# ClashLuke/LocAtE

Measured on AMD Instinct MI355X. Metric: images/sec (G+D step) 64x64 bs=64, higher is better.
Workload: dtype f32 (contractions fp32-faithful on the matrix cores: 2 x scaled fp16 operand pieces / 3 MFMAs per slice where the operand's largest magnitude comes with it, else 3 x bf16 pieces / 6 MFMAs; fp32 accumulate); 1 GPU; LocAtE G+D step, 64x64 RGB, batch 64 per GPU (the fp32 variant - the reference's own precision - of BASELINE.json configs[1]: 64x64 RGB bs 64), self/feature attention at 16x16 and 64x64, random-init weights; global_batch=64, image_size=64, parallelism=dp1, launch=hipGraph replay, G-step generator pass on a second stream

## Files before the change

### include/locate_hip.h

```cpp
#ifndef LOCATE_HIP_H
#define LOCATE_HIP_H
#include <stddef.h>
#include <stdint.h>
#ifdef __cplusplus
extern "C" {
#endif

const char* locate_last_error(void);
int locate_abi_version(void);
int locate_device_info(char* arch_name, int name_len, int* cu_count, int* wave_size);

int locate_roottanh_fwd(const float* x, float* y, int64_t n, void* absmax , void* stream);
int locate_absmax_words(void);
int locate_roottanh_bwd(const float* x, const float* gy, float* gx, int64_t n, int accumulate, void* absmax, void* stream);
int locate_absmax(const float* x, int64_t n, void* absmax, void* stream);
int locate_act_cat_rows_fwd(const float* latent, const float* pre, float* out, int rows, int z, int w, void* stream);
int locate_act_rows_bwd(const float* pre, const float* g, int64_t g_row_stride, const float* g_add, float* gpre, int rows, int w,
                        void* stream);
int locate_add3(const float* a, int64_t a_bs, const float* b, int64_t b_bs, const float* c, int64_t c_bs, float* out, int batch,
                int64_t per, void* stream);
int locate_tanh_fwd(const float* x, float* y, int64_t n, void* stream);
int locate_tanh_bwd(const float* y, const float* gy, float* gx, int64_t n, void* stream);

size_t locate_norm_stats_workspace_bytes(void);
// ... 71 lines not shown
int locate_conv_dgrad(const int* geom, const float* gy, int64_t gy_bs, const float* panel, const float* scale,
                      int scale_group_batch, int scale_stride, const float* bias, float* gx, int64_t gx_bs, void* workspace,
                      void* counters, int precision, const void* gy_absmax, const void* act_epilogue, void* stream);
size_t locate_conv_wgrad_workspace_bytes(const int* geom);
int locate_conv_wgrad_partials(const int* geom);
int locate_conv_wgrad(const int* geom, const float* x, int64_t x_bs, const float* gy, int64_t gy_bs, float* gw,
                      const float* w_ref, const float* inv_scale, int scale_group_batch, int scale_stride,
                      double* inner_partial, void* workspace, int precision, const void* x_absmax, const void* gy_absmax,
                      void* deferred_reduce, void* stream);
int locate_conv_wgrad_group_partials(const int* geom, int groups);
size_t locate_conv_wgrad_group_workspace_bytes(const int* geom, int groups);
size_t locate_slab_reduce_record_bytes(void);
int locate_slab_reduce_max(void);
int locate_slab_reduce_record_blocks(const void* record);
int locate_slab_reduce_batch(const void* records, int n, void* stream);

size_t locate_wgrad_batch_record_bytes(void);
int locate_wgrad_batch_max(void);
int locate_wgrad_batch_record(const int* geom, const float* x, int64_t x_bs, const float* gy, int64_t gy_bs, float* gw,
                              const float* w_ref, const float* inv_scale, int scale_group_batch, int scale_stride,
                              double* inner_partial, void* record);
int locate_wgrad_batch(const void* records, int n, void* stream);

int locate_dwconv_fwd(const int* geom, const float* x, int64_t x_bs, const float* w, const float* scale, int scale_group_batch,
                      int scale_stride, float* y, int64_t y_bs, void* stream);
int locate_dwconv_dgrad(const int* geom, const float* gy, int64_t gy_bs, const float* w, const float* scale,
                        int scale_group_batch, int scale_stride, float* gx, int64_t gx_bs, void* stream);
size_t locate_dwconv_wgrad_workspace_bytes(const int* geom);
int locate_dwconv_wgrad_partials(const int* geom);
int locate_dwconv_wgrad(const int* geom, const float* big, int64_t big_bs, const float* small, int64_t small_bs, float* gw,
// ... 48 lines not shown
```

### locate_amd/_lib.py

```python
import ctypes
import os

import torch

_HERE = os.path.dirname(os.path.abspath(__file__))
LIB_PATH = os.path.join(_HERE, "csrc", "liblocate_hip_dbg.so" if os.environ.get("LOCATE_HIP_DEBUG_LIBRARY") == "1"
                        else "liblocate_hip.so")

c_p = ctypes.c_void_p
c_i = ctypes.c_int
c_i64 = ctypes.c_int64
c_f = ctypes.c_float
c_d = ctypes.c_double
c_sz = ctypes.c_size_t
c_ip = ctypes.POINTER(ctypes.c_int)

PROTOTYPES = {
    "locate_last_error": (ctypes.c_char_p, []),
    "locate_abi_version": (c_i, []),
    "locate_device_info": (c_i, [ctypes.c_char_p, c_i, c_ip, c_ip]),
    "locate_roottanh_fwd": (c_i, [c_p, c_p, c_i64, c_p, c_p]),
    "locate_roottanh_bwd": (c_i, [c_p, c_p, c_p, c_i64, c_i, c_p, c_p]),
    "locate_act_cat_rows_fwd": (c_i, [c_p, c_p, c_p, c_i, c_i, c_i, c_p]),
    "locate_act_rows_bwd": (c_i, [c_p, c_p, c_i64, c_p, c_p, c_i, c_i, c_p]),
# ... 48 lines not shown
    "locate_conv_pack_panels": (c_i, [c_p, c_i, c_i, c_i, c_i, c_p]),
    "locate_conv_pack_job_is_direct": (c_i, [c_p]),
    "locate_conv_pack_job_is_window": (c_i, [c_p]),
    "locate_conv_win_ok": (c_i, [c_ip, c_i, c_i64, c_p]),
    "locate_conv_win_workspace_bytes": (c_sz, [c_ip, c_i]),
    "locate_conv_fwd_workspace_bytes": (c_sz, [c_ip]),
    "locate_conv_counter_bytes": (c_sz, []),
    "locate_conv_fwd": (c_i, [c_ip, c_p, c_i64, c_p, c_p, c_i, c_i, c_p, c_p, c_i64, c_p, c_p, c_i, c_p, c_p, c_p]),
    "locate_conv_dgrad_workspace_bytes": (c_sz, [c_ip]),
    "locate_conv_dgrad": (c_i, [c_ip, c_p, c_i64, c_p, c_p, c_i, c_i, c_p, c_p, c_i64, c_p, c_p, c_i, c_p, c_p, c_p]),
    "locate_conv_wgrad_workspace_bytes": (c_sz, [c_ip]),
    "locate_conv_wgrad_partials": (c_i, [c_ip]),
    "locate_conv_wgrad": (c_i, [c_ip, c_p, c_i64, c_p, c_i64, c_p, c_p, c_p, c_i, c_i, c_p, c_p, c_i, c_p, c_p, c_p, c_p]),
    "locate_conv_wgrad_group_partials": (c_i, [c_ip, c_i]),
    "locate_conv_wgrad_group_workspace_bytes": (c_sz, [c_ip, c_i]),
    "locate_slab_reduce_record_bytes": (c_sz, []),
    "locate_slab_reduce_max": (c_i, []),
    "locate_slab_reduce_record_blocks": (c_i, [c_p]),
    "locate_slab_reduce_batch": (c_i, [c_p, c_i, c_p]),
    "locate_dwconv_fwd": (c_i, [c_ip, c_p, c_i64, c_p, c_p, c_i, c_i, c_p, c_i64, c_p]),
    "locate_dwconv_dgrad": (c_i, [c_ip, c_p, c_i64, c_p, c_p, c_i, c_i, c_p, c_i64, c_p]),
    "locate_dwconv_wgrad_workspace_bytes": (c_sz, [c_ip]),
    "locate_dwconv_wgrad_partials": (c_i, [c_ip]),
    "locate_dwconv_wgrad": (c_i, [c_ip, c_p, c_i64, c_p, c_i64, c_p, c_p, c_p, c_i, c_i, c_p, c_p, c_p]),
    "locate_groupdot_fwd": (c_i, [c_p, c_i64, c_p, c_p, c_i, c_i, c_p, c_i, c_i, c_i, c_p]),
    "locate_groupdot_dgrad": (c_i, [c_p, c_p, c_p, c_i, c_i, c_p, c_i64, c_i, c_i, c_i, c_p]),
    "locate_groupdot_wgrad_partials": (c_i, [c_i, c_i]),
    "locate_groupdot_wgrad": (c_i, [c_p, c_i64, c_p, c_p, c_p, c_p, c_i, c_i, c_p, c_i, c_i, c_i, c_p]),
    "locate_fin_record_bytes": (c_sz, []),
    "locate_fin_sn_dot_partials": (c_i, [c_i, c_i, c_i]),
# ... 13 lines not shown
    "locate_g_loss": (c_i, [c_p, c_i, c_p, c_p, c_p]),
    "locate_input_param_record_bytes": (c_sz, []),
    "locate_input_mean_blocks": (c_i, [c_i, c_i]),
    "locate_input_workspace_bytes": (c_sz, [c_i, c_i, c_i]),
    "locate_input_transform": (c_i, [c_p, c_i, c_i, c_i, c_p, c_p, c_i, c_i, c_p, c_i, c_i, c_i, c_p, c_i, c_p, c_p, c_p, c_p]),
    "locate_image_range_workspace_bytes": (c_sz, []),
    "locate_image_range": (c_i, [c_p, c_i64, c_p, c_p, c_p]),
    "locate_image_grid": (c_i, [c_p, c_i, c_i, c_i, c_i, c_f, c_p, c_f, c_p, c_p, c_p]),
}


class LocateError(RuntimeError):
    pass


EXPECTED_ABI = 10


_lib = None


def lib():
    global _lib
    if _lib is None:
        if not os.path.exists(LIB_PATH):
            raise LocateError("%s is missing: run `python -m locate_amd.build` (hipcc, gfx950). "
                              "There is no CPU fallback for the MI355X kernels." % LIB_PATH)
        handle = ctypes.CDLL(LIB_PATH)
        for name, (res, args) in PROTOTYPES.items():
            fn = getattr(handle, name)
            fn.restype = res
# ... 26 lines not shown
```

### locate_amd/csrc/convwgrad.hip

```cpp
#include "igemm.h"

#define WG_BK 32

struct WgParams {
    const float* x;
    const float* gy;
    float* slab;
    long long x_bs, gy_bs;
    unsigned x_bytes;
    int B, C, H, W, M, OH, OW, KH, KW, stride, pad_h, pad_w;
    int R;
    int N;
    int chunk;
    int zper, Ng;
    unsigned q_mul, ow_mul;
    int q_s1, q_s2, ow_s1, ow_s2;
    int gscale_bg, gscale_stride;
    float* direct_out;
    const float* w_ref;
    const float* inv_scale;
    double* partial;
    const unsigned* x_absmax;
    const unsigned* g_absmax;
};


template <int WGM, int WGN, int TM, int TN>
__device__ __forceinline__ void wgrad_epilogue(const WgParams& p, f32x16 (&acc)[TM][TN], int r0, int m0, int wm, int wn, int lane,
                                               int wid, int tid) {
    const int lrow = lane >> 5, lcol = lane & 31;
    __shared__ double red[4];
    const bool direct = p.direct_out != nullptr;
    float* dst = direct ? p.direct_out : p.slab + (long long)blockIdx.z * p.M * p.R;
    const float sc = (direct && p.inv_scale && p.gscale_bg == 0) ? p.inv_scale[0] : 1.0f;
    double dot = 0.0;
    const bool want_dot = direct && p.w_ref != nullptr;
#pragma unroll
    for (int j = 0; j < TN; ++j) {
        const int r = r0 + (wn * TN + j) * 32 + lcol;
        const bool r_ok = r < p.R;
#pragma unroll
        for (int i = 0; i < TM; ++i) {
            float wref[16];
#pragma unroll
            for (int e = 0; e < 16; ++e) {
                const int m = m0 + (wm * TM + i) * 32 + (e & 3) + 8 * (e >> 2) + 4 * lrow;
                const bool ok = want_dot && r_ok && m < p.M;
                const float* wp_ = ok ? p.w_ref + (long long)m * p.R + r : p.gy;
// ... 2 lines not shown
            float part = 0.0f;
#pragma unroll
            for (int e = 0; e < 16; ++e) {
                const int m = m0 + (wm * TM + i) * 32 + (e & 3) + 8 * (e >> 2) + 4 * lrow;
                const float v = acc[i][j][e];
                part = fmaf(v, wref[e], part);
                if (r_ok && m < p.M) dst[(long long)m * p.R + r] = v * sc;
            }
            dot += (double)part;
        }
    }
    if (direct && p.partial) {
        dot = wave_sum_d(dot);
        if (lane == 0) red[wid] = dot;
        __syncthreads();
        if (tid == 0) p.partial[blockIdx.y * gridDim.x + blockIdx.x] = (red[0] + red[1]) + (red[2] + red[3]);
    }
}

template <int WGM, int WGN, int TM, int TN>
__global__ void __launch_bounds__(256) conv_wgrad_kernel(const WgParams p) {
    constexpr int BM = WGM * TM * 32;
    constexpr int BR = WGN * TN * 32;
    constexpr int G_PT = WG_BK * BM / 256;
    constexpr int X_PT = WG_BK * BR / 256;
    static_assert(WGM * WGN == 4, "four waves");

    __shared__ float Gs[2][WG_BK][BM + 1];
    __shared__ float Xs[2][WG_BK][BR + 1];
    __shared__ int rt_off[BR];
    __shared__ signed char rt_dy[BR], rt_dx[BR];

    const int tid = threadIdx.x, lane = tid & 63, wid = tid >> 6;
    const int wm = wid / WGN, wn = wid % WGN;
    const int r0 = blockIdx.x * BR, m0 = blockIdx.y * BM;
    const int taps = p.KH * p.KW;
    for (int i = tid; i < BR; i += 256) {
        const int r = r0 + i;
        if (r < p.R) {
            const int c = r / taps, t = r - c * taps;
            const int kh = t / p.KW, kw = t - kh * p.KW;
            rt_dy[i] = (signed char)(kh - p.pad_h);
            rt_dx[i] = (signed char)(kw - p.pad_w);
            rt_off[i] = c * p.H * p.W + (kh - p.pad_h) * p.W + (kw - p.pad_w);
        } else {
            rt_dy[i] = rt_dx[i] = 0;
// ... 90 lines not shown
        for (int k2 = 0; k2 < WG_BK / 2; ++k2) {
            float a[TM], b[TN];
#pragma unroll
            for (int i = 0; i < TM; ++i) a[i] = Gs[buf][k2 * 2 + lrow][(wm * TM + i) * 32 + lcol];
#pragma unroll
            for (int j = 0; j < TN; ++j) b[j] = Xs[buf][k2 * 2 + lrow][(wn * TN + j) * 32 + lcol];
#pragma unroll
            for (int i = 0; i < TM; ++i)
#pragma unroll
                for (int j = 0; j < TN; ++j) acc[i][j] = __builtin_amdgcn_mfma_f32_32x32x2f32(a[i], b[j], acc[i][j], 0, 0, 0);
        }
        if (s + 1 < nsteps) store_tiles(buf ^ 1);
        __syncthreads();
    }

    wgrad_epilogue<WGM, WGN, TM, TN>(p, acc, r0, m0, wm, wn, lane, wid, tid);
}

#define WB_BK 16
#define WB_PITCH 8

template <int WGM, int WGN, int TM, int TN, int NP>
__global__ void __launch_bounds__(256, (WGM * TM > 4 ? 2 : 3)) conv_wgrad_bx6_kernel(const WgParams p) {
    constexpr int BM = WGM * TM * 32;
    constexpr int BR = WGN * TN * 32;
    constexpr int G_PT = BM / 32;
    constexpr int X_PT = BR / 32;
    static_assert(WGM * WGN == 4, "four waves");

    constexpr int NPL = NP == 4 ? 1 : NP;
    __shared__ unsigned Gs[2][NPL][NP == 4 ? 1 : BM][WB_PITCH];
    __shared__ unsigned Xs[2][NPL][NP == 4 ? 1 : BR][WB_PITCH];
    __shared__ __attribute__((aligned(16))) unsigned short G8[2][NP == 4 ? BM : 1][8];
    __shared__ __attribute__((aligned(16))) unsigned short X8[2][NP == 4 ? BR : 1][8];

    const int tid = threadIdx.x, lane = tid & 63, wid = tid >> 6;
    const int wm = wid / WGN, wn = wid % WGN;
    const int r0 = blockIdx.x * BR, m0 = blockIdx.y * BM;
    const int taps = p.KH * p.KW;
    const int np = tid & 7, sub = tid >> 3;
    const int Q = p.OH * p.OW;

    int xoff[X_PT], xdy[X_PT], xdx[X_PT];
#pragma unroll
    for (int i = 0; i < X_PT; ++i) {
        const int r = r0 + sub + 32 * i;
        if (r < p.R) {
            const int c = r / taps, t = r - c * taps;
            const int kh = t / p.KW, kw = t - kh * p.KW;
            xdy[i] = kh - p.pad_h;
            xdx[i] = kw - p.pad_w;
            xoff[i] = 4 * (c * p.H * p.W + xdy[i] * p.W + xdx[i]);
        } else {
            xdy[i] = -(1 << 20);
            xdx[i] = 0;
            xoff[i] = 0;
        }
    }
    const __amdgpu_buffer_rsrc_t xrsrc = __builtin_amdgcn_make_buffer_rsrc(const_cast<float*>(p.x), 0, (int)p.x_bytes, 0x00020000);

    f32x16 acc[TM][TN];
#pragma unroll
    for (int i = 0; i < TM; ++i)
#pragma unroll
        for (int j = 0; j < TN; ++j)
#pragma unroll
            for (int r = 0; r < 16; ++r) acc[i][j][r] = 0.0f;

    const int zgrp = (int)blockIdx.z / p.zper;
    const int n_begin = zgrp * p.Ng + ((int)blockIdx.z - zgrp * p.zper) * p.chunk;
    int n_end = n_begin + p.chunk;
    if (n_end > (zgrp + 1) * p.Ng) n_end = (zgrp + 1) * p.Ng;

    float gs0 = 1.0f, gs1 = 1.0f, gs2 = 1.0f, gs3 = 1.0f, gsc = 1.0f;
    if (p.gscale_bg > 0) {
        const int ng = p.B / p.gscale_bg;
        gs0 = p.inv_scale[0];
        gs1 = ng > 1 ? p.inv_scale[p.gscale_stride] : 1.0f;
        gs2 = ng > 2 ? p.inv_scale[2 * p.gscale_stride] : 1.0f;
        gs3 = ng > 3 ? p.inv_scale[3 * p.gscale_stride] : 1.0f;
    }

    float g_scale = 1.0f, x_scale = 1.0f, g_unscale = 1.0f, x_unscale = 1.0f;
    if constexpr (NP == 2) {
        const float gmax = __uint_as_float(absmax_read(p.g_absmax)) * fmaxf(fmaxf(gs0, gs1), fmaxf(gs2, gs3));
// ... 149 lines not shown
        __builtin_amdgcn_sched_barrier(0);
        store_tiles(buf ^ 1);
        load_tiles(n_begin + (s + 2) * WB_BK);
        __builtin_amdgcn_sched_barrier(0);
        mfmas(HALF, NMF);
        __syncthreads();
    }
    if constexpr (NP == 2 || NP == 4) {
#pragma unroll
        for (int i = 0; i < TM; ++i)
#pragma unroll
            for (int j = 0; j < TN; ++j)
#pragma unroll
                for (int r = 0; r < 16; ++r) acc[i][j][r] = (acc[i][j][r] * g_unscale) * x_unscale;
    }
    wgrad_epilogue<WGM, WGN, TM, TN>(p, acc, r0, m0, wm, wn, lane, wid, tid);
}

template <int V>
__device__ __forceinline__ void slab_load(const float* p, float (&v)[V]) {
    if constexpr (V == 4) { const float4 t = *reinterpret_cast<const float4*>(p); v[0] = t.x; v[1] = t.y; v[2] = t.z; v[3] = t.w; }
    else v[0] = *p;
}

template <int ZP, int V>
__device__ __forceinline__ void slab_reduce_groups(const float* __restrict__ slab, float* __restrict__ out, int64_t n, int nsplit,
                                                   const float* __restrict__ w_ref, double* __restrict__ partial, int bid, int nblocks,
                                                   int groups, int zper, float* zbuf, double* gscratch) {
    float (*gzsum)[ZP][256 / ZP][V] = reinterpret_cast<float (*)[ZP][256 / ZP][V]>(zbuf);
    constexpr int TPB = 256 / ZP, EPB = TPB * V;
    const int ex = threadIdx.x % TPB, ez = threadIdx.x / TPB;
// ... 712 lines not shown
    return !path_disabled("skinny") && !skinny_wgrad_ok(g) && g.OH == 1 && g.OW == 1 && (long long)g.C * g.H * g.W < (1 << 24);
}
static dim3 onepix_wgrad_grid(const ConvGeom& g) { return dim3((g.C * g.H * g.W + 63) / 64, (g.M + skw_mt(g.M) - 1) / skw_mt(g.M)); }

enum WgradKind { WG_MAP1X1, WG_ONEPIX, WG_POINTWISE, WG_TILED };
struct WgradRoute {
    WgradKind kind;
    dim3 grid;
    int bm;
    PwPlan pw;
    int nsplit, chunk, zper;
    int64_t n;
    int partials;
    size_t ws_bytes;
    bool dots;
};

static WgradRoute wgrad_route(const ConvGeom& g, int groups) {
    WgradRoute r;
    const bool stacked = groups >= 2 && groups <= 4 && g.B % groups == 0;
    if (!stacked) groups = 0;
    r.bm = 0; r.nsplit = 1; r.chunk = 0; r.zper = 1; r.partials = 0; r.ws_bytes = 0; r.dots = false;
    r.n = (int64_t)g.M * g.C * g.KH * g.KW;
    const bool map1x1 = skinny_wgrad_ok(g);
    if (map1x1 || onepix_wgrad_ok(g)) {
        r.kind = map1x1 ? WG_MAP1X1 : WG_ONEPIX;
        r.grid = map1x1 ? skinny_wgrad_grid(g) : onepix_wgrad_grid(g);
        r.partials = (int)(r.grid.x * r.grid.y);
        return r;
    }
    r.pw = pw_plan(g, groups);
    if (r.pw.ok) {
        r.kind = WG_POINTWISE;
        if (stacked && r.pw.zper == 0) return r;
        r.nsplit = r.pw.nslab; r.chunk = r.pw.chunk; r.zper = r.pw.zper;
        r.grid = dim3(r.pw.nslab, r.pw.tiles_m * r.pw.tiles_c);
        r.dots = stacked;
    } else {
        r.kind = WG_TILED;
        int tiles;
        wgrad_plan(g, groups, &r.bm, &r.nsplit, &r.chunk, &r.zper, &tiles);
        r.grid = dim3((g.C * g.KH * g.KW + 127) / 128, (g.M + r.bm - 1) / r.bm, r.nsplit);
        r.dots = stacked && (long long)g.B * g.OH * g.OW < (1ll << 31);
        if (r.nsplit == 1) { r.partials = tiles; return r; }
    }
    r.partials = wgrad_reduce_grid(r.n, r.nsplit);
    r.ws_bytes = (size_t)r.nsplit * r.n * sizeof(float);
    return r;
}

LOCATE_API size_t locate_conv_wgrad_workspace_bytes(const int* geom) { return wgrad_route(make_geom(geom), 0).ws_bytes; }

LOCATE_API int locate_conv_wgrad_partials(const int* geom) { return wgrad_route(make_geom(geom), 0).partials; }

LOCATE_API size_t locate_wgrad_batch_record_bytes(void) { return sizeof(SkwRec); }
LOCATE_API int locate_wgrad_batch_max(void) { return SKW_MAX; }
LOCATE_API int locate_wgrad_batch_record(const int* geom, const float* x, int64_t x_bs, const float* gy, int64_t gy_bs, float* gw,
                                         const float* w_ref, const float* inv_scale, int scale_group_batch, int scale_stride,
// ... 39 lines not shown
    const WgradRoute r = wgrad_route(g, groups);
    return r.dots ? r.partials : 0;
}
LOCATE_API size_t locate_conv_wgrad_group_workspace_bytes(const int* geom, int groups) {
    const ConvGeom g = make_geom(geom);
    if (geom_check(g, "locate_conv_wgrad_group_workspace_bytes")) return 0;
    const WgradRoute r = wgrad_route(g, groups);
    return r.dots ? r.ws_bytes : 0;
}

template <int NP>
static void launch_wgrad_bx6(const WgParams& p, dim3 grid, int bm, hipStream_t st) {
    with_tile<true>(bm, [&](auto t) { using T = decltype(t); conv_wgrad_bx6_kernel<T::wgm, T::wgn, T::tm, T::tn, NP><<<grid, 256, 0, st>>>(p); });
}

LOCATE_API int locate_conv_wgrad(const int* geom, const float* x, int64_t x_bs, const float* gy, int64_t gy_bs, float* gw,
                                 const float* w_ref, const float* inv_scale, int scale_group_batch, int scale_stride,
                                 double* inner_partial, void* workspace, int precision, const void* x_absmax, const void* gy_absmax,
                                 void* deferred_reduce, void* stream) {
    const ConvGeom g = make_geom(geom);
    if (int e = geom_check(g, "locate_conv_wgrad")) return e;
    LOCATE_REQUIRE(precision >= 0 && precision <= 3, "locate_conv_wgrad: precision must be 0 (fp32-faithful, bf16 pieces), 1 (bf16 operands), 2 (fp32-faithful, fp16 pieces) or 3 (fp8 operands)");
    LOCATE_REQUIRE(precision < 2 || (x_absmax && gy_absmax), "locate_conv_wgrad: precisions 2 and 3 need the absmax words of x and gy");
    LOCATE_REQUIRE(x && gy && gw, "locate_conv_wgrad: null pointer");
    LOCATE_REQUIRE(!inner_partial || w_ref, "locate_conv_wgrad: inner_partial needs w_ref");
    const int gd = (scale_group_batch > 0 && w_ref && inner_partial && g.B % scale_group_batch == 0) ? g.B / scale_group_batch : 0;
    const WgradRoute r = wgrad_route(g, gd);
    LOCATE_REQUIRE(scale_group_batch >= 0 && (scale_group_batch == 0 || (inv_scale && g.B % scale_group_batch == 0 &&
                   g.B / scale_group_batch <= 4 && ((!w_ref && !inner_partial) || r.dots))),
                   "locate_conv_wgrad: bad group scaling arguments (per-call partials: see locate_conv_wgrad_group_partials)");
    hipStream_t st = as_stream(stream);
    if (deferred_reduce) memset(deferred_reduce, 0, sizeof(SlabRec));
    auto reduce = [&](const float* slab, const float* scale, const char* who) -> int {
        const int64_t n = r.n;
        const int nsplit = r.nsplit, zper = r.zper, rg = r.partials;
        const int zp = wgrad_reduce_zp(nsplit, n);
        if (deferred_reduce) {
            SlabRec rec;
            rec.slab = slab; rec.out = gw; rec.w_ref = w_ref; rec.inv_scale = scale; rec.partial = inner_partial;
            rec.n = n; rec.nsplit = nsplit; rec.zp = zp; rec.grid = rg; rec.block0 = 0; rec.groups = gd; rec.zper = zper;
            memcpy(deferred_reduce, &rec, sizeof(rec));
            return LOCATE_OK;
        }
        if (zp == 16) slab_reduce_kernel<16><<<rg, 256, 0, st>>>(slab, gw, n, nsplit, w_ref, scale, inner_partial, gd, zper);
        else if (zp == 4) slab_reduce_kernel<4><<<rg, 256, 0, st>>>(slab, gw, n, nsplit, w_ref, scale, inner_partial, gd, zper);
        else slab_reduce_kernel<1><<<rg, 256, 0, st>>>(slab, gw, n, nsplit, w_ref, scale, inner_partial, gd, zper);
        LOCATE_LAUNCH_CHECK(who);
        return LOCATE_OK;
    };
    if (r.kind == WG_MAP1X1) {
        skinny_wgrad_kernel<<<r.grid, 256, 0, st>>>(x, x_bs, gy, gy_bs, gw, w_ref, inv_scale, scale_group_batch, scale_stride,
                                                   inner_partial, g.B, g.M, g.C, OnePix{0, 0, 0, 0, 0, 0, 0});
        LOCATE_LAUNCH_CHECK("locate_conv_wgrad(1x1 map)");
        return LOCATE_OK;
    }
    if (r.kind == WG_ONEPIX) {
        const OnePix op = {g.H * g.W, g.W, g.KH, g.KW, g.pad_h, g.pad_w, g.C};
        skinny_wgrad_kernel<<<r.grid, 256, 0, st>>>(x, x_bs, gy, gy_bs, gw, w_ref, inv_scale, scale_group_batch, scale_stride,
// ... 24 lines not shown
            else pw_wgrad_kernel<2, 2, 2><<<grid, 256, 0, st>>>(q);
        } else if (precision == 1) {
            if (key == 0) pw_wgrad_kernel<1, 1, 1><<<grid, 256, 0, st>>>(q);
            else if (key == 1) pw_wgrad_kernel<1, 2, 1><<<grid, 256, 0, st>>>(q);
            else if (key == 2) pw_wgrad_kernel<2, 1, 1><<<grid, 256, 0, st>>>(q);
            else pw_wgrad_kernel<2, 2, 1><<<grid, 256, 0, st>>>(q);
        } else {
            if (key == 0) pw_wgrad_kernel<1, 1, 3><<<grid, 256, 0, st>>>(q);
            else if (key == 1) pw_wgrad_kernel<1, 2, 3><<<grid, 256, 0, st>>>(q);
            else if (key == 2) pw_wgrad_kernel<2, 1, 3><<<grid, 256, 0, st>>>(q);
            else pw_wgrad_kernel<2, 2, 3><<<grid, 256, 0, st>>>(q);
        }
        LOCATE_LAUNCH_CHECK("locate_conv_wgrad(pointwise)");
        return reduce(q.slab, grouped ? nullptr : inv_scale, "locate_conv_wgrad(pointwise reduce)");
    }
    const int bm = r.bm, nsplit = r.nsplit, chunk = r.chunk, zper = r.zper;
    LOCATE_REQUIRE(nsplit == 1 || workspace, "locate_conv_wgrad: split reduction needs a workspace");
    WgParams p;
    p.x = x; p.gy = gy; p.slab = static_cast<float*>(workspace); p.x_bs = x_bs; p.gy_bs = gy_bs;
    p.B = g.B; p.C = g.C; p.H = g.H; p.W = g.W; p.M = g.M; p.OH = g.OH; p.OW = g.OW; p.KH = g.KH; p.KW = g.KW;
    p.stride = g.stride; p.pad_h = g.pad_h; p.pad_w = g.pad_w;
    p.R = g.C * g.KH * g.KW; p.N = g.B * g.OH * g.OW; p.chunk = chunk;
    p.zper = zper; p.Ng = gd > 1 ? p.N / gd : p.N;
    fastdiv_make((unsigned)(g.OH * g.OW), &p.q_mul, &p.q_s1, &p.q_s2);
    fastdiv_make((unsigned)g.OW, &p.ow_mul, &p.ow_s1, &p.ow_s2);
    const bool direct = nsplit == 1;
    const bool grouped = scale_group_batch > 0;
    p.gscale_bg = scale_group_batch; p.gscale_stride = scale_stride;
    p.x_absmax = static_cast<const unsigned*>(x_absmax);
    p.g_absmax = static_cast<const unsigned*>(gy_absmax);
    p.direct_out = direct ? gw : nullptr;
    p.w_ref = direct ? w_ref : nullptr;
    p.inv_scale = (direct || grouped) ? inv_scale : nullptr;
    p.partial = direct ? inner_partial : nullptr;
    const long long x_extent = 4ll * ((long long)(g.B - 1) * x_bs + (long long)g.C * g.H * g.W);
    p.x_bytes = (unsigned)x_extent;
    const bool pairs_ok = ((g.OH * g.OW) & 1) == 0 && (g.OW & 1) == 0 && (gy_bs & 1) == 0 && (chunk & 1) == 0 &&
                          (reinterpret_cast<uintptr_t>(gy) & 7) == 0 && x_extent > 0 && x_extent < (1ll << 31) - (1 << 20);
    LOCATE_REQUIRE(bm != 192 || pairs_ok, "locate_conv_wgrad: layers with M %% 192 == 0 on even maps take the paired-load kernels - gy must be 8-byte aligned with an even batch stride");
    const bool bx6 = pairs_ok && (precision == 1 || precision == 3 || !path_disabled("wbx6"));
    if (bx6 && precision == 3) launch_wgrad_bx6<4>(p, grid, bm, st);
    else if (bx6 && precision == 1) launch_wgrad_bx6<1>(p, grid, bm, st);
    else if (bx6 && precision == 2) launch_wgrad_bx6<2>(p, grid, bm, st);
    else if (bx6) launch_wgrad_bx6<3>(p, grid, bm, st);
    else
        with_tile<false>(bm, [&](auto t) { using T = decltype(t); conv_wgrad_kernel<T::wgm, T::wgn, T::tm, T::tn><<<grid, 256, 0, st>>>(p); });
    LOCATE_LAUNCH_CHECK("locate_conv_wgrad(gemm)");
    if (!direct) return reduce(p.slab, grouped ? nullptr : inv_scale, "locate_conv_wgrad(reduce)");
    return LOCATE_OK;
}

LOCATE_API size_t locate_slab_reduce_record_bytes(void) { return sizeof(SlabRec); }
LOCATE_API int locate_slab_reduce_max(void) { return SLAB_MAX; }
LOCATE_API int locate_slab_reduce_record_blocks(const void* record) {
    if (!record) return 0;
    SlabRec r;
    memcpy(&r, record, sizeof(r));
    return r.grid;
}
LOCATE_API int locate_slab_reduce_batch(const void* records, int n, void* stream) {
    LOCATE_REQUIRE(records && n > 0 && n <= SLAB_MAX, "locate_slab_reduce_batch: 1 .. locate_slab_reduce_max() records");
    SlabBatch b;
    memcpy(b.r, records, (size_t)n * sizeof(SlabRec));
    long long blocks = 0;
    for (int i = 0; i < n; ++i) {
        const SlabRec& r = b.r[i];
// ... 10 lines not shown
```

### locate_amd/csrc/runtime.hip

```cpp
#include "common.h"
#include <stdarg.h>
#include <stdio.h>

static thread_local char g_last_error[512] = "";

void locate_set_error(const char* fmt, ...) {
    va_list ap;
    va_start(ap, fmt);
    vsnprintf(g_last_error, sizeof(g_last_error), fmt, ap);
    va_end(ap);
}

LOCATE_API const char* locate_last_error(void) { return g_last_error; }

LOCATE_API int locate_abi_version(void) { return 10; }

LOCATE_API int locate_device_info(char* arch_name, int name_len, int* cu_count, int* wave_size) {
    int dev = 0;
    hipDeviceProp_t prop;
    if (hipGetDevice(&dev) != hipSuccess || hipGetDeviceProperties(&prop, dev) != hipSuccess) {
        locate_set_error("locate_device_info: no HIP device");
        return LOCATE_ERR_LAUNCH;
    }
    if (arch_name && name_len > 0) snprintf(arch_name, name_len, "%s", prop.gcnArchName);
    if (cu_count) *cu_count = prop.multiProcessorCount;
    if (wave_size) *wave_size = prop.warpSize;
    return LOCATE_OK;
}
```

### locate_amd/ops.py

```python
import ctypes
import os

import torch

from ._lib import check, lib

_IntArr12 = ctypes.c_int * 12


class _ActEpilogue(ctypes.Structure):
    _fields_ = [("act_out", ctypes.c_void_p), ("act_bs", ctypes.c_int64), ("lat", ctypes.c_void_p), ("lat_bs", ctypes.c_int64),
                ("lat_z", ctypes.c_int32), ("pad", ctypes.c_int32), ("mul_pre", ctypes.c_void_p), ("mul_bs", ctypes.c_int64),
                ("out_absmax", ctypes.c_void_p)]


ACT_LINKS = [os.environ.get("LOCATE_ACT_LINKS", "1") != "0"]
ACT_LINK_MAX_NUMEL = [int(os.environ.get("LOCATE_ACT_LINK_MAX", str(1 << 22)))]


class ActLink:
    __slots__ = ("pre", "premultiplied")

    def __init__(self):
        self.pre = None
# ... 215 lines not shown

class Runtime:

    def __init__(self):
        self.precision = 0
        self.stacked = 1
        self.weight_grad_stream = None
        self.weight_grad_side_min_flops = float(os.environ.get("LOCATE_WGRAD_SIDE_MIN_GFLOP", "0")) * 1e9
        self._dv_layers = {}
        self._dv_tables = {}
        self._end_scheduled = False
        self._side = None
        self._side_results = []
        self._keep = []
        self.defer_finalisers = True
        self._fin_dots = []
        self._fin_rank1 = []
        self._fin_sums = []
        self._fin_chan = []
        self._fin_norm = []
        self._fin_wgrad = []
        self._fin_slab = []
        self._streams = {}
        self._homes_taken = set()

    def __deepcopy__(self, memo):
        rt = Runtime()
        rt.precision = self.precision
        rt.defer_finalisers = self.defer_finalisers
        return rt

    def stacked_calls(self, n):
        return _Stacked(self, n)

    def weight_grads_on(self, stream):
        return _OnStream(self, stream)

    def finalisers_deferred(self, on):
        return _Deferral(self, on)

    def reset(self):
        self._end_scheduled = False
        self._side = None
        self._side_results = []
        self._keep = []
        self._streams = {}
        self._homes_taken = set()
        AMAX.new_pass()
        self._fin_dots, self._fin_rank1, self._fin_sums, self._fin_chan, self._fin_norm = [], [], [], [], []
        self._fin_wgrad, self._fin_slab = [], []
        for entry in self._dv_layers.values():
            entry[5]["k"] = 0
        self._dv_layers = {}

    def _schedule_end(self):
        st = torch.cuda.current_stream()
        self._streams[st.cuda_stream] = st
        if not self._end_scheduled:
            torch.autograd.Variable._execution_engine.queue_callback(self._end_of_backward)
            self._end_scheduled = True

    def _end_of_backward(self):
        self._end_scheduled = False
        side, self._side = self._side, None
        cur = torch.cuda.current_stream()
        if side is not None:
            cur.wait_stream(side)
        used, self._streams = self._streams, {}
        for sid, st_ in used.items():
            if sid != cur.cuda_stream:
                cur.wait_stream(st_)
        L = lib()
        st = _stream()
        if self._fin_wgrad:
            cap = L.locate_wgrad_batch_max()
            for i in range(0, len(self._fin_wgrad), cap):
                chunk = self._fin_wgrad[i:i + cap]
                check(L.locate_wgrad_batch(b"".join(chunk), len(chunk), st), "locate_wgrad_batch")
            self._fin_wgrad = []
        if self._fin_slab:
            cap = L.locate_slab_reduce_max()
            for i in range(0, len(self._fin_slab), cap):
                chunk = self._fin_slab[i:i + cap]
                check(L.locate_slab_reduce_batch(b"".join(chunk), len(chunk), st), "locate_slab_reduce_batch")
            self._fin_slab = []
        for queue, fn, name in ((self._fin_dots, L.locate_fin_sn_dots, "locate_fin_sn_dots"),
                                (self._fin_rank1, L.locate_fin_sn_rank1, "locate_fin_sn_rank1"),
                                (self._fin_sums, L.locate_fin_sums, "locate_fin_sums"),
# ... 40 lines not shown
        hw = g.numel() // (Bn * Cn)
        slices = lib().locate_fin_channel_slices(Bn, Cn, hw)
        part = torch.empty(slices * Cn, dtype=torch.float32, device=g.device) if slices > 1 else None
        self._fin_chan.append(self._rec([g, out, part], [g.stride(0)], [Bn, Cn, hw]))
        self._keep.append((g, out, part))
        self._schedule_end()

    def queue_norm_channels(self, ws, plane_offset, planes, stats, dscale, dbias, B, C, groups):
        s1 = ws.data_ptr() + plane_offset
        self._fin_norm.append(self._rec([s1, s1 + 4 * planes, stats, dscale, dbias], [], [B, C, groups]))
        self._keep.append((ws, stats, dscale, dbias))
        self._schedule_end()

    def queue_small_wgrad(self, record, operands):
        self._fin_wgrad.append(record)
        self._keep.append(operands)
        self._schedule_end()

    def queue_slab_reduce(self, record, operands):
        self._fin_slab.append(record)
        self._keep.append(operands)
        self._schedule_end()

    def late_grad(self, param, grad):
        self._side_results.append((param, grad))
        self._schedule_end()

    def defer_dv(self, v_param, u_param, w, h, wd):
        st = v_param.__dict__.get("_locate_dv")
        if st is None or st["dv"].device != v_param.device:
# ... 821 lines not shown
        rec = ctypes.create_string_buffer(L.locate_wgrad_batch_record_bytes())
        if L.locate_wgrad_batch_record(garr, _p(xin), _bs(xin), _p(gout), _bs(gout), _p(gw), _p(w_ref), _p(inv_sigma), sbg, sst,
                                       _p(partial), rec) > 0:
            rt.queue_small_wgrad(rec.raw, (xin, gout, gw, w_ref, inv_sigma, partial))
            return
    if spec.mode == "dense":
        nbytes = L.locate_conv_wgrad_group_workspace_bytes(garr, group_dots) if group_dots else L.locate_conv_wgrad_workspace_bytes(garr)
        defer = rt is not None and rt.defer_finalisers and nbytes > 0
        ws = torch.empty(nbytes, dtype=torch.uint8, device=xin.device) if defer else _ws(nbytes, xin.device)
        rec = ctypes.create_string_buffer(L.locate_slab_reduce_record_bytes()) if defer else None
        f16 = _f16_ok(spec, geom, precision, amax_in, amax_out)
        F16_CALLS["wgrad"] += int(f16)
        if precision == 3:
            amax_in, amax_out = _ensure_amax(xin), _ensure_amax(gout)
        scaled = f16 or precision == 3
        check(L.locate_conv_wgrad(garr, _p(xin), _bs(xin), _p(gout), _bs(gout), _p(gw), _p(w_ref), _p(inv_sigma), sbg, sst, _p(partial),
                                  _p(ws), 2 if f16 else precision, _p(amax_in) if scaled else None, _p(amax_out) if scaled else None, rec, st),
              "locate_conv_wgrad")
        if defer and L.locate_slab_reduce_record_blocks(rec) > 0:
            rt.queue_slab_reduce(rec.raw, (ws, gw, w_ref, inv_sigma, partial))
    elif spec.mode == "depthwise":
        ws = _ws(L.locate_dwconv_wgrad_workspace_bytes(garr), xin.device)
        check(L.locate_dwconv_wgrad(garr, _p(xin), _bs(xin), _p(gout), _bs(gout), _p(gw), _p(w_ref), _p(inv_sigma), sbg, sst,
                                    _p(partial), _p(ws), st), "locate_dwconv_wgrad")
    else:
        B, G, Ln = geom[:3]
        gout = gout.contiguous()
        check(L.locate_groupdot_wgrad(_p(xin), _bs(xin), _p(gout), _p(gw), _p(w_ref), _p(inv_sigma), sbg, sst, _p(partial), B, G, Ln,
                                      st), "locate_groupdot_wgrad")

# ... 212 lines not shown
```

Baseline: 7132 images/sec.

## Pool small tiled conv wgrad launches into one grouped kernel at pass end

Adds a pooled wgrad kernel that takes up to 16 tiled conv weight-gradient records and runs all their blocks in a single launch, each block picking its record by block offset. Eligible small layers (bounded block count and operand size) are deferred to the end of the backward pass and grouped by operand precision form, and their slab reductions stay queued as before. The aim is fewer kernel launches and better CU fill for small wgrad GEMMs. In exchange every pooled block reserves LDS sized for the largest 128x128 tile, which can lower occupancy, and the wgrads lose overlap with the rest of the backward pass because they now wait until its end.

```diff
diff --git a/include/locate_hip.h b/include/locate_hip.h
--- a/include/locate_hip.h
+++ b/include/locate_hip.h
@@ -109,6 +109,13 @@
 int locate_slab_reduce_max(void);
 int locate_slab_reduce_record_blocks(const void* record);
 int locate_slab_reduce_batch(const void* records, int n, void* stream);
+size_t locate_wgrad_pool_record_bytes(void);
+int locate_wgrad_pool_max(void);
+int locate_wgrad_pool_record(const int* geom, const float* x, int64_t x_bs, const float* gy, int64_t gy_bs, float* gw,
+                             const float* w_ref, const float* inv_scale, int scale_group_batch, int scale_stride,
+                             double* inner_partial, void* workspace, int precision, const void* x_absmax, const void* gy_absmax,
+                             void* deferred_reduce, void* record);
+int locate_wgrad_pool(const void* records, int n, int precision, void* stream);
 
 size_t locate_wgrad_batch_record_bytes(void);
 int locate_wgrad_batch_max(void);
diff --git a/locate_amd/_lib.py b/locate_amd/_lib.py
--- a/locate_amd/_lib.py
+++ b/locate_amd/_lib.py
@@ -86,6 +86,10 @@
     "locate_conv_wgrad": (c_i, [c_ip, c_p, c_i64, c_p, c_i64, c_p, c_p, c_p, c_i, c_i, c_p, c_p, c_i, c_p, c_p, c_p, c_p]),
     "locate_conv_wgrad_group_partials": (c_i, [c_ip, c_i]),
     "locate_conv_wgrad_group_workspace_bytes": (c_sz, [c_ip, c_i]),
+    "locate_wgrad_pool_record_bytes": (c_sz, []),
+    "locate_wgrad_pool_max": (c_i, []),
+    "locate_wgrad_pool_record": (c_i, [c_ip, c_p, c_i64, c_p, c_i64, c_p, c_p, c_p, c_i, c_i, c_p, c_p, c_i, c_p, c_p, c_p, c_p]),
+    "locate_wgrad_pool": (c_i, [c_p, c_i, c_i, c_p]),
     "locate_slab_reduce_record_bytes": (c_sz, []),
     "locate_slab_reduce_max": (c_i, []),
     "locate_slab_reduce_record_blocks": (c_i, [c_p]),
@@ -129,7 +133,7 @@
     pass
 
 
-EXPECTED_ABI = 10
+EXPECTED_ABI = 11
 
 
 _lib = None
diff --git a/locate_amd/csrc/convwgrad.hip b/locate_amd/csrc/convwgrad.hip
--- a/locate_amd/csrc/convwgrad.hip
+++ b/locate_amd/csrc/convwgrad.hip
@@ -27,11 +27,10 @@
 
 template <int WGM, int WGN, int TM, int TN>
 __device__ __forceinline__ void wgrad_epilogue(const WgParams& p, f32x16 (&acc)[TM][TN], int r0, int m0, int wm, int wn, int lane,
-                                               int wid, int tid) {
+                                               int wid, int tid, int bz, int pidx, double* red) {
     const int lrow = lane >> 5, lcol = lane & 31;
-    __shared__ double red[4];
     const bool direct = p.direct_out != nullptr;
-    float* dst = direct ? p.direct_out : p.slab + (long long)blockIdx.z * p.M * p.R;
+    float* dst = direct ? p.direct_out : p.slab + (long long)bz * p.M * p.R;
     const float sc = (direct && p.inv_scale && p.gscale_bg == 0) ? p.inv_scale[0] : 1.0f;
     double dot = 0.0;
     const bool want_dot = direct && p.w_ref != nullptr;
@@ -64,7 +63,7 @@
         dot = wave_sum_d(dot);
         if (lane == 0) red[wid] = dot;
         __syncthreads();
-        if (tid == 0) p.partial[blockIdx.y * gridDim.x + blockIdx.x] = (red[0] + red[1]) + (red[2] + red[3]);
+        if (tid == 0) p.partial[pidx] = (red[0] + red[1]) + (red[2] + red[3]);
     }
 }
 
@@ -80,6 +79,7 @@
     __shared__ float Xs[2][WG_BK][BR + 1];
     __shared__ int rt_off[BR];
     __shared__ signed char rt_dy[BR], rt_dx[BR];
+    __shared__ double red[4];
 
     const int tid = threadIdx.x, lane = tid & 63, wid = tid >> 6;
     const int wm = wid / WGN, wn = wid % WGN;
@@ -200,14 +200,17 @@
         __syncthreads();
     }
 
-    wgrad_epilogue<WGM, WGN, TM, TN>(p, acc, r0, m0, wm, wn, lane, wid, tid);
+    wgrad_epilogue<WGM, WGN, TM, TN>(p, acc, r0, m0, wm, wn, lane, wid, tid, (int)blockIdx.z, (int)(blockIdx.y * gridDim.x + blockIdx.x), red);
 }
 
 #define WB_BK 16
 #define WB_PITCH 8
 
+template <int BM, int BR, int NP>
+constexpr int wgrad_bx6_lds_dwords() { return (NP == 4 ? 2 * (BM + BR) * 4 : 2 * NP * (BM + BR) * WB_PITCH) + 8; }
+
 template <int WGM, int WGN, int TM, int TN, int NP>
-__global__ void __launch_bounds__(256, (WGM * TM > 4 ? 2 : 3)) conv_wgrad_bx6_kernel(const WgParams p) {
+__device__ __forceinline__ void conv_wgrad_bx6_body(const WgParams& p, int bx, int by, int bz, int grid_x, unsigned* lds) {
     constexpr int BM = WGM * TM * 32;
     constexpr int BR = WGN * TN * 32;
     constexpr int G_PT = BM / 32;
@@ -215,14 +218,15 @@
     static_assert(WGM * WGN == 4, "four waves");
 
     constexpr int NPL = NP == 4 ? 1 : NP;
-    __shared__ unsigned Gs[2][NPL][NP == 4 ? 1 : BM][WB_PITCH];
-    __shared__ unsigned Xs[2][NPL][NP == 4 ? 1 : BR][WB_PITCH];
-    __shared__ __attribute__((aligned(16))) unsigned short G8[2][NP == 4 ? BM : 1][8];
-    __shared__ __attribute__((aligned(16))) unsigned short X8[2][NP == 4 ? BR : 1][8];
+    unsigned (*Gs)[NPL][BM][WB_PITCH] = reinterpret_cast<unsigned (*)[NPL][BM][WB_PITCH]>(lds);
+    unsigned (*Xs)[NPL][BR][WB_PITCH] = reinterpret_cast<unsigned (*)[NPL][BR][WB_PITCH]>(lds + 2 * NPL * BM * WB_PITCH);
+    unsigned short (*G8)[BM][8] = reinterpret_cast<unsigned short (*)[BM][8]>(lds);
+    unsigned short (*X8)[BR][8] = reinterpret_cast<unsigned short (*)[BR][8]>(lds + 2 * BM * 4);
+    double* red = reinterpret_cast<double*>(lds + wgrad_bx6_lds_dwords<BM, BR, NP>() - 8);
 
     const int tid = threadIdx.x, lane = tid & 63, wid = tid >> 6;
     const int wm = wid / WGN, wn = wid % WGN;
-    const int r0 = blockIdx.x * BR, m0 = blockIdx.y * BM;
+    const int r0 = bx * BR, m0 = by * BM;
     const int taps = p.KH * p.KW;
     const int np = tid & 7, sub = tid >> 3;
     const int Q = p.OH * p.OW;
@@ -253,8 +257,8 @@
 #pragma unroll
             for (int r = 0; r < 16; ++r) acc[i][j][r] = 0.0f;
 
-    const int zgrp = (int)blockIdx.z / p.zper;
-    const int n_begin = zgrp * p.Ng + ((int)blockIdx.z - zgrp * p.zper) * p.chunk;
+    const int zgrp = bz / p.zper;
+    const int n_begin = zgrp * p.Ng + (bz - zgrp * p.zper) * p.chunk;
     int n_end = n_begin + p.chunk;
     if (n_end > (zgrp + 1) * p.Ng) n_end = (zgrp + 1) * p.Ng;
 
@@ -434,7 +438,43 @@
 #pragma unroll
                 for (int r = 0; r < 16; ++r) acc[i][j][r] = (acc[i][j][r] * g_unscale) * x_unscale;
     }
-    wgrad_epilogue<WGM, WGN, TM, TN>(p, acc, r0, m0, wm, wn, lane, wid, tid);
+    wgrad_epilogue<WGM, WGN, TM, TN>(p, acc, r0, m0, wm, wn, lane, wid, tid, bz, by * grid_x + bx, red);
+}
+
+template <int WGM, int WGN, int TM, int TN, int NP>
+__global__ void __launch_bounds__(256, (WGM * TM > 4 ? 2 : 3)) conv_wgrad_bx6_kernel(const WgParams p) {
+    __shared__ __attribute__((aligned(16))) unsigned lds[wgrad_bx6_lds_dwords<WGM * TM * 32, WGN * TN * 32, NP>()];
+    conv_wgrad_bx6_body<WGM, WGN, TM, TN, NP>(p, (int)blockIdx.x, (int)blockIdx.y, (int)blockIdx.z, (int)gridDim.x, lds);
+}
+
+struct WgPoolRec {
+    WgParams p;
+    int bm;
+    int gx, gy, gz;
+    int block0;
+    int form;
+};
+#define WGP_MAX 16
+struct WgPool {
+    WgPoolRec r[WGP_MAX];
+};
+static_assert(sizeof(WgPool) + 16 <= 4096, "the pooled launch's arguments must stay under 4 KiB");
+
+template <int NP>
+__global__ void __launch_bounds__(256, 3) wgrad_pool_kernel(const WgPool b, int n) {
+    __shared__ __attribute__((aligned(16))) unsigned lds[wgrad_bx6_lds_dwords<128, 128, NP>()];
+    int k = 0;
+    for (int i = 1; i < n; ++i)
+        if ((int)blockIdx.x >= b.r[i].block0) k = i;
+    const WgPoolRec& r = b.r[k];
+    const int local = (int)blockIdx.x - r.block0;
+    const int plane = r.gx * r.gy;
+    const int bz = local / plane, rem = local - bz * plane;
+    const int by = rem / r.gx, bx = rem - by * r.gx;
+    if (r.bm == 128) conv_wgrad_bx6_body<2, 2, 2, 2, NP>(r.p, bx, by, bz, r.gx, lds);
+    else if (r.bm == 96) conv_wgrad_bx6_body<1, 4, 3, 1, NP>(r.p, bx, by, bz, r.gx, lds);
+    else if (r.bm == 64) conv_wgrad_bx6_body<1, 4, 2, 1, NP>(r.p, bx, by, bz, r.gx, lds);
+    else conv_wgrad_bx6_body<1, 4, 1, 1, NP>(r.p, bx, by, bz, r.gx, lds);
 }
 
 template <int V>
@@ -1177,13 +1217,25 @@
     int partials;
     size_t ws_bytes;
     bool dots;
+    bool pool;
 };
+
+#define WGP_MAX_BLOCKS 768
+#define WGP_MAX_OPERAND_BYTES (32ll << 20)
+static bool wgrad_pool_ok(const ConvGeom& g, int bm, dim3 grid) {
+    if (path_disabled("wgpool") || path_disabled("wbx6")) return false;
+    if (bm > 128 || ((g.OH * g.OW) & 1) != 0 || (g.OW & 1) != 0) return false;
+    const long long blocks = (long long)grid.x * grid.y * grid.z;
+    const long long bytes = 4ll * ((long long)g.B * g.C * g.H * g.W + (long long)g.B * g.M * g.OH * g.OW);
+    return blocks <= knob_int("LOCATE_WGPOOL_MAX_BLOCKS", WGP_MAX_BLOCKS) &&
+           bytes <= ((long long)knob_int("LOCATE_WGPOOL_MAX_MB", (int)(WGP_MAX_OPERAND_BYTES >> 20)) << 20);
+}
 
 static WgradRoute wgrad_route(const ConvGeom& g, int groups) {
     WgradRoute r;
     const bool stacked = groups >= 2 && groups <= 4 && g.B % groups == 0;
     if (!stacked) groups = 0;
-    r.bm = 0; r.nsplit = 1; r.chunk = 0; r.zper = 1; r.partials = 0; r.ws_bytes = 0; r.dots = false;
+    r.bm = 0; r.nsplit = 1; r.chunk = 0; r.zper = 1; r.partials = 0; r.ws_bytes = 0; r.dots = false; r.pool = false;
     r.n = (int64_t)g.M * g.C * g.KH * g.KW;
     const bool map1x1 = skinny_wgrad_ok(g);
     if (map1x1 || onepix_wgrad_ok(g)) {
@@ -1205,6 +1257,7 @@
         wgrad_plan(g, groups, &r.bm, &r.nsplit, &r.chunk, &r.zper, &tiles);
         r.grid = dim3((g.C * g.KH * g.KW + 127) / 128, (g.M + r.bm - 1) / r.bm, r.nsplit);
         r.dots = stacked && (long long)g.B * g.OH * g.OW < (1ll << 31);
+        r.pool = wgrad_pool_ok(g, r.bm, r.grid);
         if (r.nsplit == 1) { r.partials = tiles; return r; }
     }
     r.partials = wgrad_reduce_grid(r.n, r.nsplit);
@@ -1274,6 +1327,42 @@
     with_tile<true>(bm, [&](auto t) { using T = decltype(t); conv_wgrad_bx6_kernel<T::wgm, T::wgn, T::tm, T::tn, NP><<<grid, 256, 0, st>>>(p); });
 }
 
+static bool wgrad_tiled_params(const ConvGeom& g, const WgradRoute& r, int gd, const float* x, int64_t x_bs, const float* gy, int64_t gy_bs,
+                               float* gw, const float* w_ref, const float* inv_scale, int scale_group_batch, int scale_stride,
+                               double* inner_partial, void* workspace, const void* x_absmax, const void* gy_absmax, WgParams* out) {
+    WgParams p;
+    p.x = x; p.gy = gy; p.slab = static_cast<float*>(workspace); p.x_bs = x_bs; p.gy_bs = gy_bs;
+    p.B = g.B; p.C = g.C; p.H = g.H; p.W = g.W; p.M = g.M; p.OH = g.OH; p.OW = g.OW; p.KH = g.KH; p.KW = g.KW;
+    p.stride = g.stride; p.pad_h = g.pad_h; p.pad_w = g.pad_w;
+    p.R = g.C * g.KH * g.KW; p.N = g.B * g.OH * g.OW; p.chunk = r.chunk;
+    p.zper = r.zper; p.Ng = gd > 1 ? p.N / gd : p.N;
+    fastdiv_make((unsigned)(g.OH * g.OW), &p.q_mul, &p.q_s1, &p.q_s2);
+    fastdiv_make((unsigned)g.OW, &p.ow_mul, &p.ow_s1, &p.ow_s2);
+    const bool direct = r.nsplit == 1;
+    const bool grouped = scale_group_batch > 0;
+    p.gscale_bg = scale_group_batch; p.gscale_stride = scale_stride;
+    p.x_absmax = static_cast<const unsigned*>(x_absmax);
+    p.g_absmax = static_cast<const unsigned*>(gy_absmax);
+    p.direct_out = direct ? gw : nullptr;
+    p.w_ref = direct ? w_ref : nullptr;
+    p.inv_scale = (direct || grouped) ? inv_scale : nullptr;
+    p.partial = direct ? inner_partial : nullptr;
+    const long long x_extent = 4ll * ((long long)(g.B - 1) * x_bs + (long long)g.C * g.H * g.W);
+    p.x_bytes = (unsigned)x_extent;
+    *out = p;
+    return ((g.OH * g.OW) & 1) == 0 && (g.OW & 1) == 0 && (gy_bs & 1) == 0 && (r.chunk & 1) == 0 &&
+           (reinterpret_cast<uintptr_t>(gy) & 7) == 0 && x_extent > 0 && x_extent < (1ll << 31) - (1 << 20);
+}
+
+static void wgrad_slab_record(const WgradRoute& r, int gd, const float* slab, float* gw, const float* w_ref, const float* scale,
+                              double* inner_partial, void* record) {
+    SlabRec rec;
+    rec.slab = slab; rec.out = gw; rec.w_ref = w_ref; rec.inv_scale = scale; rec.partial = inner_partial;
+    rec.n = r.n; rec.nsplit = r.nsplit; rec.zp = wgrad_reduce_zp(r.nsplit, r.n); rec.grid = r.partials; rec.block0 = 0; rec.groups = gd;
+    rec.zper = r.zper;
+    memcpy(record, &rec, sizeof(rec));
+}
+
 LOCATE_API int locate_conv_wgrad(const int* geom, const float* x, int64_t x_bs, const float* gy, int64_t gy_bs, float* gw,
                                  const float* w_ref, const float* inv_scale, int scale_group_batch, int scale_stride,
                                  double* inner_partial, void* workspace, int precision, const void* x_absmax, const void* gy_absmax,
@@ -1292,16 +1381,13 @@
     hipStream_t st = as_stream(stream);
     if (deferred_reduce) memset(deferred_reduce, 0, sizeof(SlabRec));
     auto reduce = [&](const float* slab, const float* scale, const char* who) -> int {
+        if (deferred_reduce) {
+            wgrad_slab_record(r, gd, slab, gw, w_ref, scale, inner_partial, deferred_reduce);
+            return LOCATE_OK;
+        }
         const int64_t n = r.n;
         const int nsplit = r.nsplit, zper = r.zper, rg = r.partials;
         const int zp = wgrad_reduce_zp(nsplit, n);
-        if (deferred_reduce) {
-            SlabRec rec;
-            rec.slab = slab; rec.out = gw; rec.w_ref = w_ref; rec.inv_scale = scale; rec.partial = inner_partial;
-            rec.n = n; rec.nsplit = nsplit; rec.zp = zp; rec.grid = rg; rec.block0 = 0; rec.groups = gd; rec.zper = zper;
-            memcpy(deferred_reduce, &rec, sizeof(rec));
-            return LOCATE_OK;
-        }
         if (zp == 16) slab_reduce_kernel<16><<<rg, 256, 0, st>>>(slab, gw, n, nsplit, w_ref, scale, inner_partial, gd, zper);
         else if (zp == 4) slab_reduce_kernel<4><<<rg, 256, 0, st>>>(slab, gw, n, nsplit, w_ref, scale, inner_partial, gd, zper);
         else slab_reduce_kernel<1><<<rg, 256, 0, st>>>(slab, gw, n, nsplit, w_ref, scale, inner_partial, gd, zper);
@@ -1356,29 +1442,13 @@
         LOCATE_LAUNCH_CHECK("locate_conv_wgrad(pointwise)");
         return reduce(q.slab, grouped ? nullptr : inv_scale, "locate_conv_wgrad(pointwise reduce)");
     }
-    const int bm = r.bm, nsplit = r.nsplit, chunk = r.chunk, zper = r.zper;
+    const int bm = r.bm, nsplit = r.nsplit;
     LOCATE_REQUIRE(nsplit == 1 || workspace, "locate_conv_wgrad: split reduction needs a workspace");
     WgParams p;
-    p.x = x; p.gy = gy; p.slab = static_cast<float*>(workspace); p.x_bs = x_bs; p.gy_bs = gy_bs;
-    p.B = g.B; p.C = g.C; p.H = g.H; p.W = g.W; p.M = g.M; p.OH = g.OH; p.OW = g.OW; p.KH = g.KH; p.KW = g.KW;
-    p.stride = g.stride; p.pad_h = g.pad_h; p.pad_w = g.pad_w;
-    p.R = g.C * g.KH * g.KW; p.N = g.B * g.OH * g.OW; p.chunk = chunk;
-    p.zper = zper; p.Ng = gd > 1 ? p.N / gd : p.N;
-    fastdiv_make((unsigned)(g.OH * g.OW), &p.q_mul, &p.q_s1, &p.q_s2);
-    fastdiv_make((unsigned)g.OW, &p.ow_mul, &p.ow_s1, &p.ow_s2);
+    const bool pairs_ok = wgrad_tiled_params(g, r, gd, x, x_bs, gy, gy_bs, gw, w_ref, inv_scale, scale_group_batch, scale_stride,
+                                             inner_partial, workspace, x_absmax, gy_absmax, &p);
     const bool direct = nsplit == 1;
     const bool grouped = scale_group_batch > 0;
-    p.gscale_bg = scale_group_batch; p.gscale_stride = scale_stride;
-    p.x_absmax = static_cast<const unsigned*>(x_absmax);
-    p.g_absmax = static_cast<const unsigned*>(gy_absmax);
-    p.direct_out = direct ? gw : nullptr;
-    p.w_ref = direct ? w_ref : nullptr;
-    p.inv_scale = (direct || grouped) ? inv_scale : nullptr;
-    p.partial = direct ? inner_partial : nullptr;
-    const long long x_extent = 4ll * ((long long)(g.B - 1) * x_bs + (long long)g.C * g.H * g.W);
-    p.x_bytes = (unsigned)x_extent;
-    const bool pairs_ok = ((g.OH * g.OW) & 1) == 0 && (g.OW & 1) == 0 && (gy_bs & 1) == 0 && (chunk & 1) == 0 &&
-                          (reinterpret_cast<uintptr_t>(gy) & 7) == 0 && x_extent > 0 && x_extent < (1ll << 31) - (1 << 20);
     LOCATE_REQUIRE(bm != 192 || pairs_ok, "locate_conv_wgrad: layers with M %% 192 == 0 on even maps take the paired-load kernels - gy must be 8-byte aligned with an even batch stride");
     const bool bx6 = pairs_ok && (precision == 1 || precision == 3 || !path_disabled("wbx6"));
     if (bx6 && precision == 3) launch_wgrad_bx6<4>(p, grid, bm, st);
@@ -1392,6 +1462,58 @@
     return LOCATE_OK;
 }
 
+LOCATE_API size_t locate_wgrad_pool_record_bytes(void) { return sizeof(WgPoolRec); }
+LOCATE_API int locate_wgrad_pool_max(void) { return WGP_MAX; }
+LOCATE_API int locate_wgrad_pool_record(const int* geom, const float* x, int64_t x_bs, const float* gy, int64_t gy_bs, float* gw,
+                                        const float* w_ref, const float* inv_scale, int scale_group_batch, int scale_stride,
+                                        double* inner_partial, void* workspace, int precision, const void* x_absmax, const void* gy_absmax,
+                                        void* deferred_reduce, void* record) {
+    const ConvGeom g = make_geom(geom);
+    if (geom_check(g, "locate_wgrad_pool_record") || !record || !x || !gy || !gw) return 0;
+    if (precision < 0 || precision > 3 || (precision >= 2 && !(x_absmax && gy_absmax))) return 0;
+    if (inner_partial && !w_ref) return 0;
+    const int gd = (scale_group_batch > 0 && w_ref && inner_partial && g.B % scale_group_batch == 0) ? g.B / scale_group_batch : 0;
+    const WgradRoute r = wgrad_route(g, gd);
+    if (r.kind != WG_TILED || !r.pool) return 0;
+    if (scale_group_batch < 0 || (scale_group_batch > 0 && !(inv_scale && g.B % scale_group_batch == 0 && g.B / scale_group_batch <= 4 &&
+                                                            ((!w_ref && !inner_partial) || r.dots)))) return 0;
+    if (r.nsplit > 1 && !(workspace && deferred_reduce)) return 0;
+    WgPoolRec rec;
+    if (!wgrad_tiled_params(g, r, gd, x, x_bs, gy, gy_bs, gw, w_ref, inv_scale, scale_group_batch, scale_stride, inner_partial, workspace,
+                            x_absmax, gy_absmax, &rec.p)) return 0;
+    rec.bm = r.bm; rec.gx = (int)r.grid.x; rec.gy = (int)r.grid.y; rec.gz = (int)r.grid.z; rec.block0 = 0; rec.form = precision;
+    if (deferred_reduce) {
+        memset(deferred_reduce, 0, sizeof(SlabRec));
+        if (r.nsplit > 1) wgrad_slab_record(r, gd, rec.p.slab, gw, w_ref, scale_group_batch > 0 ? nullptr : inv_scale, inner_partial, deferred_reduce);
+    }
+    memcpy(record, &rec, sizeof(rec));
+    return rec.gx * rec.gy * rec.gz;
+}
+LOCATE_API int locate_wgrad_pool(const void* records, int n, int precision, void* stream) {
+    LOCATE_REQUIRE(records && n > 0 && n <= WGP_MAX, "locate_wgrad_pool: 1 .. locate_wgrad_pool_max() records");
+    LOCATE_REQUIRE(precision >= 0 && precision <= 3, "locate_wgrad_pool: precision must be 0 .. 3");
+    WgPool b;
+    memcpy(b.r, records, (size_t)n * sizeof(WgPoolRec));
+    long long blocks = 0;
+    for (int i = 0; i < n; ++i) {
+        const WgPoolRec& r = b.r[i];
+        LOCATE_REQUIRE(r.p.x && r.p.gy && (r.p.slab || r.p.direct_out) && r.gx > 0 && r.gy > 0 && r.gz > 0 &&
+                       (r.bm == 128 || r.bm == 96 || r.bm == 64 || r.bm == 32) && r.p.zper > 0 && r.p.chunk > 0,
+                       "locate_wgrad_pool: bad record");
+        LOCATE_REQUIRE(r.form == precision, "locate_wgrad_pool: records of different operand forms go to separate launches");
+        b.r[i].block0 = (int)blocks;
+        blocks += (long long)r.gx * r.gy * r.gz;
+    }
+    LOCATE_REQUIRE(blocks < (1ll << 31), "locate_wgrad_pool: too many blocks");
+    hipStream_t st = as_stream(stream);
+    if (precision == 3) wgrad_pool_kernel<4><<<(unsigned)blocks, 256, 0, st>>>(b, n);
+    else if (precision == 1) wgrad_pool_kernel<1><<<(unsigned)blocks, 256, 0, st>>>(b, n);
+    else if (precision == 2) wgrad_pool_kernel<2><<<(unsigned)blocks, 256, 0, st>>>(b, n);
+    else wgrad_pool_kernel<3><<<(unsigned)blocks, 256, 0, st>>>(b, n);
+    LOCATE_LAUNCH_CHECK("locate_wgrad_pool");
+    return LOCATE_OK;
+}
+
 LOCATE_API size_t locate_slab_reduce_record_bytes(void) { return sizeof(SlabRec); }
 LOCATE_API int locate_slab_reduce_max(void) { return SLAB_MAX; }
 LOCATE_API int locate_slab_reduce_record_blocks(const void* record) {
diff --git a/locate_amd/csrc/runtime.hip b/locate_amd/csrc/runtime.hip
--- a/locate_amd/csrc/runtime.hip
+++ b/locate_amd/csrc/runtime.hip
@@ -13,7 +13,7 @@
 
 LOCATE_API const char* locate_last_error(void) { return g_last_error; }
 
-LOCATE_API int locate_abi_version(void) { return 10; }
+LOCATE_API int locate_abi_version(void) { return 11; }
 
 LOCATE_API int locate_device_info(char* arch_name, int name_len, int* cu_count, int* wave_size) {
     int dev = 0;
diff --git a/locate_amd/ops.py b/locate_amd/ops.py
--- a/locate_amd/ops.py
+++ b/locate_amd/ops.py
@@ -253,6 +253,7 @@
         self._side_results = []
         self._keep = []
         self.defer_finalisers = True
+        self.pool_wgrads = True
         self._fin_dots = []
         self._fin_rank1 = []
         self._fin_sums = []
@@ -260,6 +261,7 @@
         self._fin_norm = []
         self._fin_wgrad = []
         self._fin_slab = []
+        self._fin_pool = {}
         self._streams = {}
         self._homes_taken = set()
 
@@ -267,6 +269,7 @@
         rt = Runtime()
         rt.precision = self.precision
         rt.defer_finalisers = self.defer_finalisers
+        rt.pool_wgrads = self.pool_wgrads
         return rt
 
     def stacked_calls(self, n):
@@ -287,7 +290,7 @@
         self._homes_taken = set()
         AMAX.new_pass()
         self._fin_dots, self._fin_rank1, self._fin_sums, self._fin_chan, self._fin_norm = [], [], [], [], []
-        self._fin_wgrad, self._fin_slab = [], []
+        self._fin_wgrad, self._fin_slab, self._fin_pool = [], [], {}
         for entry in self._dv_layers.values():
             entry[5]["k"] = 0
         self._dv_layers = {}
@@ -311,6 +314,13 @@
                 cur.wait_stream(st_)
         L = lib()
         st = _stream()
+        if self._fin_pool:
+            cap = L.locate_wgrad_pool_max()
+            for form, recs in sorted(self._fin_pool.items()):
+                for i in range(0, len(recs), cap):
+                    chunk = recs[i:i + cap]
+                    check(L.locate_wgrad_pool(b"".join(chunk), len(chunk), form, st), "locate_wgrad_pool")
+            self._fin_pool = {}
         if self._fin_wgrad:
             cap = L.locate_wgrad_batch_max()
             for i in range(0, len(self._fin_wgrad), cap):
@@ -381,6 +391,11 @@
 
     def queue_small_wgrad(self, record, operands):
         self._fin_wgrad.append(record)
+        self._keep.append(operands)
+        self._schedule_end()
+
+    def queue_pooled_wgrad(self, record, form, operands):
+        self._fin_pool.setdefault(form, []).append(record)
         self._keep.append(operands)
         self._schedule_end()
 
@@ -1232,6 +1247,16 @@
         if precision == 3:
             amax_in, amax_out = _ensure_amax(xin), _ensure_amax(gout)
         scaled = f16 or precision == 3
+        form = 2 if f16 else precision
+        if rt is not None and rt.defer_finalisers and rt.pool_wgrads:
+            prec = ctypes.create_string_buffer(L.locate_wgrad_pool_record_bytes())
+            if L.locate_wgrad_pool_record(garr, _p(xin), _bs(xin), _p(gout), _bs(gout), _p(gw), _p(w_ref), _p(inv_sigma), sbg, sst,
+                                          _p(partial), _p(ws), form, _p(amax_in) if scaled else None, _p(amax_out) if scaled else None,
+                                          rec, prec) > 0:
+                rt.queue_pooled_wgrad(prec.raw, form, (xin, gout, gw, ws, w_ref, inv_sigma, partial, amax_in, amax_out))
+                if defer and L.locate_slab_reduce_record_blocks(rec) > 0:
+                    rt.queue_slab_reduce(rec.raw, (ws, gw, w_ref, inv_sigma, partial))
+                return
         check(L.locate_conv_wgrad(garr, _p(xin), _bs(xin), _p(gout), _bs(gout), _p(gw), _p(w_ref), _p(inv_sigma), sbg, sst, _p(partial),
                                   _p(ws), 2 if f16 else precision, _p(amax_in) if scaled else None, _p(amax_out) if scaled else None, rec, st),
               "locate_conv_wgrad")
```

Result: no change. 7172 images/sec (median of 6 runs) (+0.6%).
